# yerfor/Real3DPortrait

Measured on AMD Instinct MI355X. Metric: rendered frames/sec @ 512x512, 48 depth samples, higher is better.
Workload: dtype f32 operands as fp16 hi + lo, fp32 accumulate (SR precision 'f16mx' = the library default, superresolution.DEFAULT_SR_PRECISION; the fp32-class f16x3 is `alt_f16x3`): in block0.conv1, block1.conv0 and block1.conv1 hi*hi runs on the f16 MFMA and the two cross products on the block-scaled 8-bit MFMA

## Files before the change

### real3dportrait_amd/csrc/r3d_render.hip

```cpp

#include <algorithm>
#include "r3d_common.h"
#include "r3d_stamps.h"

namespace r3d {

static constexpr int kC = R3D_FEATURES;
static constexpr int kHid = R3D_HIDDEN;
static constexpr int kOut = R3D_DECODER_OUT;
static constexpr int kWavesPerBlock = 4;

__device__ __forceinline__ void block_absmax_store(float m, float* __restrict__ absmax_part, int block_linear, float* red)
{
#pragma unroll
    for (int d = 32; d >= 1; d >>= 1) m = fmaxf(m, __shfl_xor(m, d));
    const int tid = threadIdx.y * blockDim.x + threadIdx.x, nw = (blockDim.x * blockDim.y) >> 6;
    if ((tid & 63) == 0) red[tid >> 6] = m;
    __syncthreads();
    if (tid == 0) {
        float r = red[0];
        for (int w = 1; w < nw; ++w) r = fmaxf(r, red[w]);
        absmax_part[block_linear] = r;
    }
}
// ... 260 lines not shown
    if ((threadIdx.x & 63) == 0) { red[0][threadIdx.x >> 6] = kmin; red[1][threadIdx.x >> 6] = kmax; red[2][threadIdx.x >> 6] = any ? 1 : 0; }
    __syncthreads();
    if (threadIdx.x == 0) {
        int* p = gstate + kStateHeader + 3 * blockIdx.x;
        p[0] = min(min(red[0][0], red[0][1]), min(red[0][2], red[0][3]));
        p[1] = max(max(red[1][0], red[1][1]), max(red[1][2], red[1][3]));
        p[2] = red[2][0] | red[2][1] | red[2][2] | red[2][3];
    }
}

__device__ __forceinline__ void split8(const float (&x)[8], h8& hi, h8& lo)
{
#pragma unroll
    for (int j = 0; j < 8; ++j) {
        const float v = as_rounded(x[j]);
        const _Float16 a = (_Float16)fminf(fmaxf(v, -65504.f), 65504.f);
        hi[j] = a; lo[j] = (_Float16)(v - (float)a);
    }
}
__device__ __forceinline__ void split8_bounded(const float (&x)[8], h8& hi, h8& lo)
{
#pragma unroll
    for (int j = 0; j < 8; ++j) {
        const float v = as_rounded(x[j]);
        const _Float16 a = (_Float16)v;
        hi[j] = a; lo[j] = (_Float16)(v - (float)a);
    }
}

struct DecoderLds {
    uint4 w1f[4][2][64];
    uint4 w2f[2][2][2][64];
    float w2s[kHid];
    float b1[kHid];
    float b2[kOut];
    float xs3, hs, ys;
};

__device__ __forceinline__ void stage_decoder(DecoderLds& L, const float* __restrict__ w1,
                                              const float* __restrict__ b1, const float* __restrict__ w2,
                                              const float* __restrict__ b2, const DecFold* __restrict__ fold)
{
    const DecFold F = *fold;
    const float kLog2e = 1.4426950408889634f, kLn2 = 0.6931471805599453f;
    const float g1 = 0.17677669529663687f * kLog2e * F.w1s;
    const float g2 = 0.125f;
    const float g2c = g2 * F.w2s;
    for (int i = threadIdx.x; i < 4 * 64; i += blockDim.x) {
        const int l = i & 63, mt = i >> 6;
        float v[8];
#pragma unroll
        for (int j = 0; j < 8; ++j) v[j] = w1[(16 * mt + (l & 15)) * kC + 8 * (l >> 4) + j] * g1;
        h8 hi, lo; split8(v, hi, lo);
        L.w1f[mt][0][l] = *reinterpret_cast<uint4*>(&hi); L.w1f[mt][1][l] = *reinterpret_cast<uint4*>(&lo);
    }
    for (int i = threadIdx.x; i < 2 * 2 * 64; i += blockDim.x) {
        const int l = i & 63, pp = (i >> 6) & 1, ot = i >> 7;
        float v[8];
#pragma unroll
        for (int j = 0; j < 8; ++j)
            v[j] = w2[(1 + 16 * ot + (l & 15)) * kHid + 16 * (2 * pp + (j >> 2)) + 4 * (l >> 4) + (j & 3)] * g2c;
        h8 hi, lo; split8(v, hi, lo);
        L.w2f[ot][pp][0][l] = *reinterpret_cast<uint4*>(&hi); L.w2f[ot][pp][1][l] = *reinterpret_cast<uint4*>(&lo);
    }
    for (int i = threadIdx.x; i < kHid; i += blockDim.x) { L.w2s[i] = w2[i] * (g2 * kLn2); L.b1[i] = b1[i] * kLog2e; }
    for (int i = threadIdx.x; i < kOut; i += blockDim.x) L.b2[i] = i == 0 ? b2[i] : b2[i] * kLog2e * F.b2s;
    if (threadIdx.x == 0) { L.xs3 = F.xs * (1.0f / 3.0f); L.hs = F.hs; L.ys = F.ys; }
}

struct Tap { int idx; float w; };

__device__ __forceinline__ void plane_taps(float u, float v, int H, int W, int plane_base4, Tap t[4])
{
    const float ix = ((u + 1.0f) * (float)W - 1.0f) * 0.5f;
    const float iy = ((v + 1.0f) * (float)H - 1.0f) * 0.5f;
    const float x0f = floorf(ix), y0f = floorf(iy);
    const float fx1 = ix - x0f, fy1 = iy - y0f;
    const float fx0 = (x0f + 1.0f) - ix, fy0 = (y0f + 1.0f) - iy;
    const float xc = fminf(fmaxf(x0f, -2.0f), (float)W + 1.0f);
    const float yc = fminf(fmaxf(y0f, -2.0f), (float)H + 1.0f);
    const int x0 = (int)xc, y0 = (int)yc;
    const bool okc = (xc == x0f) && (yc == y0f);
    const bool vx0 = okc && x0 >= 0 && x0 < W, vx1 = okc && x0 + 1 >= 0 && x0 + 1 < W;
    const bool vy0 = okc && y0 >= 0 && y0 < H, vy1 = okc && y0 + 1 >= 0 && y0 + 1 < H;
    const int xa = min(max(x0, 0), W - 1), xb = min(max(x0 + 1, 0), W - 1);
    const int ya = min(max(y0, 0), H - 1), yb = min(max(y0 + 1, 0), H - 1);
    const int ra = __mul24(ya, W), rb = __mul24(yb, W);
    t[0].idx = plane_base4 + (ra + xa) * 8; t[0].w = (vx0 && vy0) ? fx0 * fy0 : 0.0f;
    t[1].idx = plane_base4 + (ra + xb) * 8; t[1].w = (vx1 && vy0) ? fx1 * fy0 : 0.0f;
    t[2].idx = plane_base4 + (rb + xa) * 8; t[2].w = (vx0 && vy1) ? fx0 * fy1 : 0.0f;
    t[3].idx = plane_base4 + (rb + xb) * 8; t[3].w = (vx1 && vy1) ? fx1 * fy1 : 0.0f;
}

template <int PLANES_IN_FLIGHT, bool TRI = false>
__device__ __forceinline__ void gather_sample(const float4* __restrict__ planes4, int H, int W, int q,
                                              float px, float py, float pz, float scale, float xs3, float x[8], int D = 1)
{
    const float qx = px * scale, qy = py * scale, qz = pz * scale;
    const int HW8 = H * W * 8;
    const float us[3] = {qx, qx, qz}, vs[3] = {qy, qz, qx};
    if constexpr (TRI) {
        const float ws[3] = {qz, qy, qy};
        float accs[3][8];
#pragma unroll
        for (int p = 0; p < 3; ++p)
#pragma unroll
            for (int c = 0; c < 8; ++c) accs[p][c] = 0.0f;
#pragma unroll
        for (int dz = 0; dz < 2; ++dz) {
            Tap t[12];
#pragma unroll
            for (int p = 0; p < 3; ++p) {
                const float iz = ((ws[p] + 1.0f) * (float)D - 1.0f) * 0.5f;
                const float z0f = floorf(iz);
                const float zc = fminf(fmaxf(z0f, -2.0f), (float)D + 1.0f);
                const int z = (int)zc + dz;
                const bool vz = (zc == z0f) && z >= 0 && z < D;
                const float wz = vz ? (dz ? iz - z0f : (z0f + 1.0f) - iz) : 0.0f;
                plane_taps(us[p], vs[p], H, W, (p * D + min(max(z, 0), D - 1)) * HW8 + 2 * q, t + 4 * p);
#pragma unroll
                for (int k = 0; k < 4; ++k) t[4 * p + k].w *= wz;
            }
            float4 lo[12], hi[12];
#pragma unroll
            for (int i = 0; i < 12; ++i) { lo[i] = planes4[t[i].idx]; hi[i] = planes4[t[i].idx + 1]; }
#pragma unroll
            for (int p = 0; p < 3; ++p)
#pragma unroll
                for (int k = 0; k < 4; ++k) {
                    const float w = t[4 * p + k].w;
                    const float4 a = lo[4 * p + k], b = hi[4 * p + k];
                    accs[p][0] += a.x * w; accs[p][1] += a.y * w; accs[p][2] += a.z * w; accs[p][3] += a.w * w;
                    accs[p][4] += b.x * w; accs[p][5] += b.y * w; accs[p][6] += b.z * w; accs[p][7] += b.w * w;
                }
            __builtin_amdgcn_sched_barrier(0);
        }
#pragma unroll
        for (int c = 0; c < 8; ++c) x[c] = (accs[0][c] + accs[1][c] + accs[2][c]) * xs3;
        return;
    }
    float acc[3][8];
    if (PLANES_IN_FLIGHT == 3) {
        Tap t[12];
#pragma unroll
        for (int p = 0; p < 3; ++p) plane_taps(us[p], vs[p], H, W, p * HW8 + 2 * q, t + 4 * p);
        float4 lo[12], hi[12];
#pragma unroll
        for (int i = 0; i < 12; ++i) { lo[i] = planes4[t[i].idx]; hi[i] = planes4[t[i].idx + 1]; }
#pragma unroll
        for (int p = 0; p < 3; ++p) {
#pragma unroll
            for (int c = 0; c < 8; ++c) acc[p][c] = 0.0f;
#pragma unroll
            for (int k = 0; k < 4; ++k) {
                const float w = t[4 * p + k].w;
                const float4 a = lo[4 * p + k], b = hi[4 * p + k];
                acc[p][0] += a.x * w; acc[p][1] += a.y * w; acc[p][2] += a.z * w; acc[p][3] += a.w * w;
                acc[p][4] += b.x * w; acc[p][5] += b.y * w; acc[p][6] += b.z * w; acc[p][7] += b.w * w;
            }
        }
    } else {
        const float4* __restrict__ pl = planes4 + 2 * q;
        const int pq = q < 2 ? q : 2;
        Tap tq[4];
        plane_taps(pq == 2 ? qz : qx, pq == 0 ? qy : (pq == 1 ? qz : qx), H, W, pq * HW8, tq);
#pragma unroll
        for (int p = 0; p < 3; ++p) {
            Tap t[4];
#pragma unroll
            for (int k = 0; k < 4; ++k) {
                t[k].idx = p == 0 ? __builtin_amdgcn_mov_dpp(tq[k].idx, 0x00, 0xF, 0xF, true) : p == 1 ? __builtin_amdgcn_mov_dpp(tq[k].idx, 0x55, 0xF, 0xF, true) : __builtin_amdgcn_mov_dpp(tq[k].idx, 0xAA, 0xF, 0xF, true);
                const int wi = __builtin_bit_cast(int, tq[k].w);
                t[k].w = __builtin_bit_cast(float, p == 0 ? __builtin_amdgcn_mov_dpp(wi, 0x00, 0xF, 0xF, true) : p == 1 ? __builtin_amdgcn_mov_dpp(wi, 0x55, 0xF, 0xF, true) : __builtin_amdgcn_mov_dpp(wi, 0xAA, 0xF, 0xF, true));
            }
            float4 lo[4], hi[4];
#pragma unroll
            for (int i = 0; i < 4; ++i) { lo[i] = pl[t[i].idx]; hi[i] = pl[t[i].idx + 1]; }
#pragma unroll
            for (int c = 0; c < 8; ++c) acc[p][c] = 0.0f;
#pragma unroll
            for (int k = 0; k < 4; ++k) {
                const float w = t[k].w;
                const float4 a = lo[k], b = hi[k];
                acc[p][0] += a.x * w; acc[p][1] += a.y * w; acc[p][2] += a.z * w; acc[p][3] += a.w * w;
                acc[p][4] += b.x * w; acc[p][5] += b.y * w; acc[p][6] += b.z * w; acc[p][7] += b.w * w;
            }
            __builtin_amdgcn_sched_barrier(0);
        }
    }
#pragma unroll
    for (int c = 0; c < 8; ++c) x[c] = (acc[0][c] + acc[1][c] + acc[2][c]) * xs3;
}

struct DecodeState { f32x4 h[4]; };

__device__ __forceinline__ void decode_a(const DecoderLds& L, int lane, const h8 xh, const h8 xl, DecodeState& S, float& sig)
{
    const int q = lane >> 4;
#pragma unroll
    for (int mt = 0; mt < 4; ++mt) {
        f32x4 acc;
        acc[0] = L.b1[16 * mt + 4 * q + 0]; acc[1] = L.b1[16 * mt + 4 * q + 1];
        acc[2] = L.b1[16 * mt + 4 * q + 2]; acc[3] = L.b1[16 * mt + 4 * q + 3];
        uint4 a0 = L.w1f[mt][0][lane], a1 = L.w1f[mt][1][lane];
        const h8 wh = *reinterpret_cast<h8*>(&a0), wl = *reinterpret_cast<h8*>(&a1);
        acc = __builtin_amdgcn_mfma_f32_16x16x32_f16(wl, xh, acc, 0, 0, 0);
        acc = __builtin_amdgcn_mfma_f32_16x16x32_f16(wh, xl, acc, 0, 0, 0);
        acc = __builtin_amdgcn_mfma_f32_16x16x32_f16(wh, xh, acc, 0, 0, 0);
        S.h[mt] = acc;
    }
    float sg = 0.0f;
#pragma unroll
    for (int mt = 0; mt < 4; ++mt)
#pragma unroll
        for (int r = 0; r < 4; ++r) {
            const float x = S.h[mt][r];
            const float sp = __builtin_fmaf(x + fabsf(x), 0.5f, __builtin_amdgcn_logf(1.0f + __builtin_amdgcn_exp2f(-fabsf(x))));
            S.h[mt][r] = sp;
            sg += sp * L.w2s[16 * mt + 4 * q + r];
        }
    sg += __shfl_xor(sg, 16);
    sg += __shfl_xor(sg, 32);
    sig = sg + L.b2[0];
    const float hs = L.hs;
    if (hs != 1.0f) {
#pragma unroll
        for (int mt = 0; mt < 4; ++mt)
#pragma unroll
            for (int r = 0; r < 4; ++r) S.h[mt][r] *= hs;
    }
}

template <int PP>
__device__ __forceinline__ void decode_l2(const DecoderLds& L, int lane, const DecodeState& S, f32x4 (&col)[2])
{
    const int q = lane >> 4;
    if (PP == 0) {
#pragma unroll
        for (int ot = 0; ot < 2; ++ot) {
            col[ot][0] = L.b2[1 + 16 * ot + 4 * q + 0]; col[ot][1] = L.b2[1 + 16 * ot + 4 * q + 1];
            col[ot][2] = L.b2[1 + 16 * ot + 4 * q + 2]; col[ot][3] = L.b2[1 + 16 * ot + 4 * q + 3];
        }
    }
    const float hv[8] = {S.h[2 * PP][0], S.h[2 * PP][1], S.h[2 * PP][2], S.h[2 * PP][3],
                         S.h[2 * PP + 1][0], S.h[2 * PP + 1][1], S.h[2 * PP + 1][2], S.h[2 * PP + 1][3]};
    h8 bh, bl;
    split8_bounded(hv, bh, bl);
#pragma unroll
    for (int ot = 0; ot < 2; ++ot) {
        uint4 a0 = L.w2f[ot][PP][0][lane], a1 = L.w2f[ot][PP][1][lane];
        const h8 wh = *reinterpret_cast<h8*>(&a0), wl = *reinterpret_cast<h8*>(&a1);
        col[ot] = __builtin_amdgcn_mfma_f32_16x16x32_f16(wl, bh, col[ot], 0, 0, 0);
        col[ot] = __builtin_amdgcn_mfma_f32_16x16x32_f16(wh, bl, col[ot], 0, 0, 0);
        col[ot] = __builtin_amdgcn_mfma_f32_16x16x32_f16(wh, bh, col[ot], 0, 0, 0);
    }
    if (PP == 1) {
        const float ys = L.ys;
        if (ys != 1.0f) {
#pragma unroll
            for (int ot = 0; ot < 2; ++ot)
#pragma unroll
                for (int r = 0; r < 4; ++r) col[ot][r] *= ys;
        }
#pragma unroll
        for (int ot = 0; ot < 2; ++ot)
#pragma unroll
            for (int r = 0; r < 4; ++r)
                col[ot][r] = __builtin_amdgcn_rcpf(1.0f + __builtin_amdgcn_exp2f(-col[ot][r])) * 1.002f - 0.001f;
    }
}

__device__ __forceinline__ void decode_tile(const DecoderLds& L, int lane, const h8 xh, const h8 xl, f32x4 (&col)[2], float& sig)
{
    DecodeState S;
    decode_a(L, lane, xh, xl, S, sig);
    decode_l2<0>(L, lane, S, col);
    decode_l2<1>(L, lane, S, col);
}

template <int CTRL, int ROW_MASK = 0xF>
__device__ __forceinline__ float dpp_f(float old, float x) {
    return __builtin_bit_cast(float, __builtin_amdgcn_update_dpp(__builtin_bit_cast(int, old), __builtin_bit_cast(int, x), CTRL, ROW_MASK, 0xF, false));
}
template <int CTRL, int ROW_MASK = 0xF>
__device__ __forceinline__ int dpp_i(int old, int x) { return __builtin_amdgcn_update_dpp(old, x, CTRL, ROW_MASK, 0xF, false); }
__device__ __forceinline__ float wave_incl_mul(float v, int) {
    v *= dpp_f<0x111>(1.0f, v); v *= dpp_f<0x112>(1.0f, v); v *= dpp_f<0x114>(1.0f, v); v *= dpp_f<0x118>(1.0f, v);
    v *= dpp_f<0x142, 0xA>(1.0f, v); v *= dpp_f<0x143, 0xC>(1.0f, v);
    return v;
}
__device__ __forceinline__ float wave_incl_add(float v, int) {
    v += dpp_f<0x111>(0.0f, v); v += dpp_f<0x112>(0.0f, v); v += dpp_f<0x114>(0.0f, v); v += dpp_f<0x118>(0.0f, v);
    v += dpp_f<0x142, 0xA>(0.0f, v); v += dpp_f<0x143, 0xC>(0.0f, v);
    return v;
}
__device__ __forceinline__ int wave_incl_add_i(int v) {
    v += dpp_i<0x111>(0, v); v += dpp_i<0x112>(0, v); v += dpp_i<0x114>(0, v); v += dpp_i<0x118>(0, v);
    v += dpp_i<0x142, 0xA>(0, v); v += dpp_i<0x143, 0xC>(0, v);
    return v;
}
__device__ __forceinline__ float wave_shift_up1(float v, float first) { return dpp_f<0x138>(first, v); }
__device__ __forceinline__ float lane63(float v) { return __builtin_bit_cast(float, __builtin_amdgcn_readlane(__builtin_bit_cast(int, v), 63)); }
__device__ __forceinline__ float wave_sum(float v) { return lane63(wave_incl_add(v, 0)); }
__device__ __forceinline__ void wave_lds_sync() {
    __builtin_amdgcn_fence(__ATOMIC_ACQ_REL, "wavefront");
    __builtin_amdgcn_wave_barrier();
}

struct XchLds { uint4 v[2][64]; };
__device__ __forceinline__ int gather_q(int lane) { return lane & 3; }
__device__ __forceinline__ int gather_s(int lane) { return lane >> 2; }
__device__ __forceinline__ void gather_to_mfma(XchLds& E, int lane, const float (&X)[8], h8& xh, h8& xl)
{
    split8_bounded(X, xh, xl);
    const int gs = lane >> 2, gq = lane & 3, q = lane >> 4, s = lane & 15;
    const int wi = 16 * gq + (gs ^ (2 * gq)), ri = 16 * q + (s ^ (2 * q));
    E.v[0][wi] = *reinterpret_cast<uint4*>(&xh);
    E.v[1][wi] = *reinterpret_cast<uint4*>(&xl);
    wave_lds_sync();
    uint4 rh = E.v[0][ri], rl = E.v[1][ri];
    wave_lds_sync();
    xh = *reinterpret_cast<h8*>(&rh);
    xl = *reinterpret_cast<h8*>(&rl);
}

template <int NS, int NCD>
struct RayLds {
    float t[NS];
    float sg[NS];
    float ts[NS];
    float ss[NS];
    float wv[NS];
    float om[NS];
    float cdf[NCD];
    int cnt[NS];
};

struct FeatLds { uint4 v[2][2 * 64]; };

typedef __amdgpu_buffer_rsrc_t PlaneRsrc;
template <int NB = 2>
struct TileGather {
    f32x4 lo[NB][4], hi[NB][4];
    float tw[NB][4];
    Tap tq[4];
    float acc[8];
    __device__ __forceinline__ void start(int H, int W, int q, float px, float py, float pz, float scale)
    {
        const float qx = px * scale, qy = py * scale, qz = pz * scale;
        const int pq = q < 2 ? q : 2;
        plane_taps(pq == 2 ? qz : qx, pq == 0 ? qy : (pq == 1 ? qz : qx), H, W, pq * H * W * 8, tq);
#pragma unroll
        for (int k = 0; k < 4; ++k) tq[k].idx *= 16;
    }
    template <int P, int B>
    __device__ __forceinline__ void issue(const PlaneRsrc rsrc, unsigned qoff)
    {
#pragma unroll
        for (int k = 0; k < 4; ++k) {
            const int wbits = __builtin_bit_cast(int, tq[k].w);
            const unsigned off = (unsigned)(P == 0 ? __builtin_amdgcn_mov_dpp(tq[k].idx, 0x00, 0xF, 0xF, true) : P == 1 ? __builtin_amdgcn_mov_dpp(tq[k].idx, 0x55, 0xF, 0xF, true) : __builtin_amdgcn_mov_dpp(tq[k].idx, 0xAA, 0xF, 0xF, true)) + qoff;
            tw[B][k] = __builtin_bit_cast(float, P == 0 ? __builtin_amdgcn_mov_dpp(wbits, 0x00, 0xF, 0xF, true) : P == 1 ? __builtin_amdgcn_mov_dpp(wbits, 0x55, 0xF, 0xF, true) : __builtin_amdgcn_mov_dpp(wbits, 0xAA, 0xF, 0xF, true));
            lo[B][k] = __builtin_bit_cast(f32x4, __builtin_amdgcn_raw_buffer_load_b128(rsrc, (int)off, 0, 0));
            hi[B][k] = __builtin_bit_cast(f32x4, __builtin_amdgcn_raw_buffer_load_b128(rsrc, (int)(off + 16u), 0, 0));
        }
    }
    template <int B>
    __device__ __forceinline__ void pin(f32x4& d0, f32x4& d1)
    {
        asm volatile("" : "+v"(lo[B][0]), "+v"(lo[B][1]), "+v"(lo[B][2]), "+v"(lo[B][3]), "+v"(hi[B][0]), "+v"(hi[B][1]), "+v"(hi[B][2]), "+v"(hi[B][3]),
                          "+v"(d0), "+v"(d1));
    }
    template <int P, int B>
    __device__ __forceinline__ void consume()
    {
        float pa[8];
#pragma unroll
        for (int c = 0; c < 8; ++c) pa[c] = 0.0f;
#pragma unroll
        for (int k = 0; k < 4; ++k) {
            const float w = tw[B][k];
            const f32x4 a4 = lo[B][k], b4 = hi[B][k];
            pa[0] += a4[0] * w; pa[1] += a4[1] * w; pa[2] += a4[2] * w; pa[3] += a4[3] * w;
            pa[4] += b4[0] * w; pa[5] += b4[1] * w; pa[6] += b4[2] * w; pa[7] += b4[3] * w;
        }
#pragma unroll
        for (int c = 0; c < 8; ++c) acc[c] = P == 0 ? pa[c] : acc[c] + pa[c];
    }
    __device__ __forceinline__ void finish(FeatLds& F, int slot, int wi, float xs3)
    {
        float X[8];
#pragma unroll
        for (int c = 0; c < 8; ++c) X[c] = acc[c] * xs3;
        h8 xh, xl;
        split8_bounded(X, xh, xl);
        F.v[0][slot * 64 + wi] = *reinterpret_cast<uint4*>(&xh);
        F.v[1][slot * 64 + wi] = *reinterpret_cast<uint4*>(&xl);
    }
};

template <int NT, int GPF, bool TRI, int NB = 2, typename DepthFn, typename FirstFn>
__device__ __forceinline__ void decode_pass(FeatLds& F, const DecoderLds& dec, const float4* __restrict__ P, int H, int W, int D, int lane,
                                            float ox, float oy, float oz, float dx, float dy, float dz, float scale, float xs3,
                                            DepthFn depth_of, FirstFn first_done, f32x4 (&col0)[NT], f32x4 (&col1)[NT], float (&sig)[NT], f32x4* gp = nullptr)
{
    const int gq = lane & 3, gs = lane >> 2, q = lane >> 4, s = lane & 15;
    const int wi = 16 * gq + (gs ^ (2 * gq)), ri = 16 * q + (s ^ (2 * q));
    const uint64_t pb = (uint64_t)(uintptr_t)P;
    void* pu = reinterpret_cast<void*>((uintptr_t)(((uint64_t)(unsigned)__builtin_amdgcn_readfirstlane((int)(pb >> 32)) << 32) |
                                                   (unsigned)__builtin_amdgcn_readfirstlane((int)(pb & 0xffffffffu))));
    const PlaneRsrc pl = __builtin_amdgcn_make_buffer_rsrc(pu, 0, __builtin_amdgcn_readfirstlane(3 * (TRI ? D : 1) * H * W * 128), 0x00020000);
    const unsigned qoff = 32u * (unsigned)gq;
    TileGather<NB> g;
    auto gather_whole = [&](int t) {
        const float tg = depth_of(t);
        if constexpr (TRI) {
            float X[8]; h8 xh, xl;
            gather_sample<GPF, true>(P, H, W, gq, ox + tg * dx, oy + tg * dy, oz + tg * dz, scale, xs3, X, D);
            split8_bounded(X, xh, xl);
            F.v[0][(t & 1) * 64 + wi] = *reinterpret_cast<uint4*>(&xh); F.v[1][(t & 1) * 64 + wi] = *reinterpret_cast<uint4*>(&xl);
        } else {
            f32x4 z0 = {0.f, 0.f, 0.f, 0.f}, z1 = z0;
            g.start(H, W, gq, ox + tg * dx, oy + tg * dy, oz + tg * dz, scale);
            g.template issue<0, 0>(pl, qoff);
            if constexpr (NB == 2) {
                g.template issue<1, 1>(pl, qoff);
                g.template pin<0>(z0, z1); g.template consume<0, 0>();
                g.template issue<2, 0>(pl, qoff);
                g.template pin<1>(z0, z1); g.template consume<1, 1>();
                g.template pin<0>(z0, z1); g.template consume<2, 0>();
            } else {
                g.template pin<0>(z0, z1); g.template consume<0, 0>();
                g.template issue<1, 0>(pl, qoff);
                g.template pin<0>(z0, z1); g.template consume<1, 0>();
                g.template issue<2, 0>(pl, qoff);
                g.template pin<0>(z0, z1); g.template consume<2, 0>();
            }
            g.finish(F, t & 1, wi, xs3);
        }
    };
    gather_whole(0);
    first_done();
#pragma unroll
    for (int t = 0; t < NT; ++t) {
        wave_lds_sync();
        uint4 rh = F.v[0][(t & 1) * 64 + ri], rl4 = F.v[1][(t & 1) * 64 + ri];
        const h8 xh = *reinterpret_cast<h8*>(&rh), xl = *reinterpret_cast<h8*>(&rl4);
        const bool more = t + 1 < NT;
        DecodeState S;
        f32x4 c2[2];
        if (more && !TRI) {
            const float tg = depth_of(t + 1);
            g.start(H, W, gq, ox + tg * dx, oy + tg * dy, oz + tg * dz, scale);
            g.template issue<0, 0>(pl, qoff);
        }
        __builtin_amdgcn_sched_barrier(0);
        decode_a(dec, lane, xh, xl, S, sig[t]);
        __builtin_amdgcn_sched_barrier(0);
        if (more && !TRI) { g.template pin<0>(S.h[0], S.h[3]); g.template consume<0, 0>(); g.template issue<1, 0>(pl, qoff); }
        __builtin_amdgcn_sched_barrier(0);
        decode_l2<0>(dec, lane, S, c2);
        __builtin_amdgcn_sched_barrier(0);
        if (more && !TRI) { g.template pin<0>(c2[0], c2[1]); g.template consume<1, 0>(); g.template issue<2, 0>(pl, qoff); }
        __builtin_amdgcn_sched_barrier(0);
        decode_l2<1>(dec, lane, S, c2);
        __builtin_amdgcn_sched_barrier(0);
        if (more && !TRI) { g.template pin<0>(c2[0], c2[1]); g.template consume<2, 0>(); g.finish(F, (t + 1) & 1, wi, xs3); }
        if (more && TRI) gather_whole(t + 1);
        if (gp) { gp[(2 * t) * 64] = c2[0]; gp[(2 * t + 1) * 64] = c2[1]; }
        else { col0[t] = c2[0]; col1[t] = c2[1]; }
        __builtin_amdgcn_sched_barrier(0);
    }
}

template <int SLOTS>
__device__ __forceinline__ void march(const float* T, const float* S, float* wv, int n, int lane,
                                      float& wsum, float& dsum)
{
    float carry = 1.0f, ws = 0.0f, ds = 0.0f;
#pragma unroll
    for (int sl = 0; sl < SLOTS; ++sl) {
        const int i = sl * 64 + lane;
        const bool act = i < n - 1;
        const int i0 = act ? i : 0;
        const float t0 = T[i0], t1 = T[i0 + 1], s0 = S[i0], s1 = S[i0 + 1];
        const float delta = t1 - t0;
        const float dmid = (s0 + s1) * 0.5f;
        const float tmid = (t0 + t1) * 0.5f;
        const float sp = softplus20(dmid - 1.0f);
        const float alpha = one_minus_exp_neg(sp * delta);
        const float om1 = act ? (1.0f - alpha + 1e-10f) : 1.0f;
        const float incl = wave_incl_mul(om1, lane);
        const float excl = wave_shift_up1(incl, 1.0f);
        const float w = act ? alpha * (carry * excl) : 0.0f;
        carry *= lane63(incl);
        if (act) wv[i] = w;
        ws += w;
        ds += w * tmid;
    }
    wsum = wave_sum(ws);
    dsum = wave_sum(ds);
}

constexpr bool render_shape_parks(int ntc, int ntf) { return ntf > 0 && ntc > 3; }
constexpr int render_park_tiles(int ntc, int ntf) { return render_shape_parks(ntc, ntf) ? 2 * (ntc + ntf) : 0; }

struct RenderArgs {
    const float4* planes4; int N, H, W, M, D;
    const float* w1; const float* b1; const float* w2; const float* b2;
    const float* origins; const float* dirs;
    const float* cam_c2w; const float* cam_K; int cam_R;
    uint2* split_out; const float* split_scale; size_t split_scale_stride;
    const float* ray_start; const float* ray_end; const uint8_t* valid;
    int* gstate; int nlimit_blocks;
    int Nc, Nf; float scale; int white_back;
    const float* noise_c; const float* u_f; unsigned long long seed;
    const DecFold* fold;
    float* rgb; float* depth; float* wsum; int rgb_cm;
    unsigned long long* clk;
    f32x4* park_g;
};

struct RayIter {
    int strips, n, c, row, sa, sb, sc, R, strip, N, M, col0;
    long long lin, lstride, nrays;
    __device__ __forceinline__ void init(const RenderArgs& a, int R_, int wave)
    {
        const int wv = __builtin_amdgcn_readfirstlane(wave);
        R = R_; N = a.N; M = a.M;
        strips = (R > 0 && (R & 7) == 0 && (gridDim.x & 7) == 0) ? 1 : 0;
        if (strips) {
            const unsigned xcd = blockIdx.x & 7, bx = blockIdx.x >> 3, nbx = gridDim.x >> 3;
            strip = R >> 3; col0 = (int)xcd * strip;
            const unsigned per_img = (unsigned)strip * (unsigned)R;
            const unsigned w0 = bx * kWavesPerBlock + (unsigned)wv, st = nbx * kWavesPerBlock;
            n = (int)(w0 / per_img); const unsigned rem = w0 - (unsigned)n * per_img;
            c = (int)(rem / (unsigned)R); row = (int)(rem - (unsigned)c * (unsigned)R);
            sa = (int)(st / per_img); const unsigned srem = st - (unsigned)sa * per_img;
            sb = (int)(srem / (unsigned)R); sc = (int)(srem - (unsigned)sb * (unsigned)R);
        } else {
            nrays = (long long)a.N * a.M;
            lin = (long long)blockIdx.x * kWavesPerBlock + wv;
            lstride = (long long)gridDim.x * kWavesPerBlock;
        }
    }
    __device__ __forceinline__ bool get(int& ray, int& img) const
    {
        if (strips) { if (n >= N) return false; img = n; ray = n * M + row * R + col0 + c; return true; }
        if (lin >= nrays) return false;
        ray = (int)lin; img = ray / M; return true;
    }
    __device__ __forceinline__ void advance()
    {
        if (strips) {
            row += sc; if (row >= R) { row -= R; ++c; }
            c += sb;   if (c >= strip) { c -= strip; ++n; }
            n += sa;
        } else lin += lstride;
    }
};

template <int NTC, int NTF, int OCC, int GPF, bool TRI = false>
__global__ __launch_bounds__(256, OCC) void render_kernel(RenderArgs a, int R)
{
    constexpr int SLOTS = (16 * (NTC + NTF) + 63) / 64;
    constexpr int CSLOTS = (16 * NTC + 63) / 64;
    constexpr int FSLOTS = NTF > 0 ? (16 * NTF + 63) / 64 : 1;
    typedef RayLds<16 * (NTC + NTF) + 8, 16 * NTC + 8> RayL;
    __shared__ __attribute__((aligned(16))) DecoderLds dec;
    __shared__ __attribute__((aligned(16))) RayL rl[kWavesPerBlock];
    __shared__ __attribute__((aligned(16))) FeatLds feat[kWavesPerBlock];
    constexpr bool PARK = NTF > 0 && NTC <= 3;
    constexpr bool GPARK = render_shape_parks(NTC, NTF);
    __shared__ __attribute__((aligned(16))) f32x4 park[PARK ? kWavesPerBlock : 1][PARK ? 2 * NTC : 1][64];

    stage_decoder(dec, a.w1, a.b1, a.w2, a.b2, a.fold);
    __syncthreads();
    const float xs3 = dec.xs3;

    const int lane = threadIdx.x & 63, wave = threadIdx.x >> 6;
    const int q = lane >> 4, s = lane & 15;
    const int gs = gather_s(lane);
    RayL& L = rl[wave];
    FeatLds& F = feat[wave];
    int pmin = 0x7fffffff, pmax = (int)0x80000000, pany = 0;
    for (int b = lane; b < a.nlimit_blocks; b += 64) {
        const int* p = a.gstate + kStateHeader + 3 * b;
        pmin = min(pmin, p[0]); pmax = max(pmax, p[1]); pany |= p[2];
    }
#pragma unroll
    for (int d = 32; d >= 1; d >>= 1) { pmin = min(pmin, __shfl_xor(pmin, d)); pmax = max(pmax, __shfl_xor(pmax, d)); pany |= __shfl_xor(pany, d); }
    const float gmin_start = ord2f(pmin), gmax_start = ord2f(pmax);
    const bool any_valid = pany != 0;
    const int Nc_all = a.Nc;
    float run_min = INFINITY, run_max = -INFINITY;
    R3D_STAMP_DECL;
    int st_rays_ = 0; (void)st_rays_;
    if (blockIdx.x == (gridDim.x >> 1) && threadIdx.x == 0) clk_begin(kernarg_clk<RenderArgs>());

    RayIter it;
    it.init(a, R, wave);
    for (;; it.advance()) {
        typedef const __attribute__((address_space(4))) RenderArgs* KArgs;
        KArgs ap = (KArgs)__builtin_amdgcn_kernarg_segment_ptr();
        asm volatile("" : "+s"(ap));
        const auto& A = *ap;
        const int Nc = NTF > 0 ? A.Nc : Nc_all, Nf = A.Nf, S = Nc + Nf;
        int ray, n;
        if (!it.get(ray, n)) break;
        ++st_rays_;
        R3D_STAMP(7);
        const float4* P = A.planes4 + (size_t)n * 3 * (TRI ? A.D : 1) * A.H * A.W * 8;
        float ox, oy, oz, dx, dy, dz;
        if (A.cam_c2w) {
            float o3[3], d3[3];
            make_ray(A.cam_c2w + 16 * n, A.cam_K + 9 * n, A.cam_R, ray - n * A.M, o3, d3);
            ox = o3[0]; oy = o3[1]; oz = o3[2]; dx = d3[0]; dy = d3[1]; dz = d3[2];
        } else {
            ox = A.origins[3 * (size_t)ray]; oy = A.origins[3 * (size_t)ray + 1]; oz = A.origins[3 * (size_t)ray + 2];
            dx = A.dirs[3 * (size_t)ray]; dy = A.dirs[3 * (size_t)ray + 1]; dz = A.dirs[3 * (size_t)ray + 2];
        }
        float start = A.ray_start[ray], end = A.ray_end[ray];
        if (!A.valid[ray] && any_valid) { start = gmin_start; end = gmax_start; }

        const float span = end - start;
        const float delta = span / (float)(Nc - 1);
        float tc[NTC];
#pragma unroll
        for (int nt = 0; nt < NTC; ++nt) {
            const int k = 16 * nt + s;
            const bool act = k < Nc;
            const float step = (float)k / (float)(Nc - 1);
            float u = 0.0f;
            if (act) u = A.noise_c ? A.noise_c[(size_t)ray * Nc + k] : hash_uniform(A.seed, 0, (uint64_t)ray * Nc + k);
            tc[nt] = act ? (start + step * span) + u * delta : start;
        }
        R3D_STAMP(0);
        f32x4 colc[2][NTC];
        float sigc[NTC];
        f32x4* gpark = nullptr;
        if constexpr (GPARK) gpark = A.park_g + ((size_t)(blockIdx.x * kWavesPerBlock + wave) * render_park_tiles(NTC, NTF)) * 64 + lane;
        {
            if (q == 0) {
#pragma unroll
                for (int nt = 0; nt < NTC; ++nt) {
                    const int k = 16 * nt + s;
                    if (k < Nc) L.t[k] = tc[nt];
                }
            }
            wave_lds_sync();
            auto dof = [&](int t) { const int k = 16 * t + gs; return k < Nc ? L.t[k] : start; };
            decode_pass<NTC, GPF, TRI, (OCC >= 3 ? 1 : 2)>(F, dec, P, A.H, A.W, A.D, lane, ox, oy, oz, dx, dy, dz, A.scale, xs3, dof,
                                                           [&]() { R3D_STAMP(8); }, colc[0], colc[1], sigc, gpark);
        }
        constexpr bool parked = PARK;
        if (parked) {
#pragma unroll
            for (int nt = 0; nt < NTC; ++nt) { park[PARK ? wave : 0][PARK ? 2 * nt : 0][lane] = colc[0][nt]; park[PARK ? wave : 0][PARK ? 2 * nt + 1 : 0][lane] = colc[1][nt]; }
        }

        if (q == 0) {
#pragma unroll
            for (int nt = 0; nt < NTC; ++nt) {
                const int k = 16 * nt + s;
                if (k < Nc) L.sg[k] = sigc[nt];
            }
        }
        wave_lds_sync();
        R3D_STAMP(1);

        float wsum, dsum;
        f32x4 colf[2][NTF > 0 ? NTF : 1];
        bool fine_done = false;
        if constexpr (NTF > 0) { if (Nf > 0) {
            fine_done = true;
            march<CSLOTS>(L.t, L.sg, L.wv, Nc, lane, wsum, dsum);
            wave_lds_sync();
            const int ns = Nc - 3;
            float omega[CSLOTS], tot = 0.0f;
#pragma unroll
            for (int sl = 0; sl < CSLOTS; ++sl) {
                const int i = sl * 64 + lane;
                const bool act = i < ns;
                const int i0 = act ? i : 0;
                const float w0 = L.wv[i0], w1v = L.wv[i0 + 1], w2v = L.wv[i0 + 2];
                const float sv = (fmaxf(w0, w1v) + fmaxf(w1v, w2v)) * 0.5f + 0.01f;
                omega[sl] = act ? sv + 1e-5f : 0.0f;
                tot += omega[sl];
            }
            tot = wave_sum(tot);
            float carry = 0.0f;
            if (lane == 0) L.cdf[0] = 0.0f;
#pragma unroll
            for (int sl = 0; sl < CSLOTS; ++sl) {
                const int i = sl * 64 + lane;
                const float incl = wave_incl_add(omega[sl] / tot, lane);
                if (i < ns) L.cdf[i + 1] = carry + incl;
                carry += lane63(incl);
            }
            wave_lds_sync();
#pragma unroll
            for (int sl = 0; sl < FSLOTS; ++sl) {
                const int j = sl * 64 + lane;
                if (j < Nf) {
                    const float u = A.u_f ? A.u_f[(size_t)ray * Nf + j] : hash_uniform(A.seed, 1, (uint64_t)ray * Nf + j);
                    int lo = 0, hi = ns + 1;
                    while (lo < hi) { const int mid = (lo + hi) >> 1; if (L.cdf[mid] <= u) lo = mid + 1; else hi = mid; }
                    const int below = max(lo - 1, 0), above = min(lo, ns);
                    const float cb = L.cdf[below], ca = L.cdf[above];
                    const float bb = 0.5f * (L.t[below] + L.t[below + 1]);
                    const float ba = 0.5f * (L.t[above] + L.t[above + 1]);
                    float den = ca - cb;
                    if (den < 1e-5f) den = 1.0f;
                    L.t[Nc + j] = bb + (u - cb) / den * (ba - bb);
                }
            }
            wave_lds_sync();
            R3D_STAMP(2);
            float sigf[NTF > 0 ? NTF : 1];
            {
                auto dof = [&](int t) { const int k = 16 * t + gs; return L.t[Nc + (k < Nf ? k : 0)]; };
                decode_pass<(NTF > 0 ? NTF : 1), GPF, TRI, (OCC >= 3 ? 1 : 2)>(F, dec, P, A.H, A.W, A.D, lane, ox, oy, oz, dx, dy, dz, A.scale, xs3, dof,
                                                                             [&]() { R3D_STAMP(9); }, colf[0], colf[1], sigf, GPARK ? gpark + 2 * NTC * 64 : nullptr);
            }
            if (q == 0) {
#pragma unroll
                for (int nt = 0; nt < NTF; ++nt) {
                    const int k = 16 * nt + s;
                    if (k < Nf) L.sg[Nc + k] = sigf[nt];
                }
            }
            wave_lds_sync();
            R3D_STAMP(3);
            int rank[SLOTS];
            bool fast = true;
#pragma unroll
            for (int sl = 0; sl < CSLOTS; ++sl) {
                const int i = sl * 64 + lane;
                const bool act = i < Nc - 1;
                fast = fast && (!act || L.t[act ? i : 0] <= L.t[act ? i + 1 : 0]);
            }
            fast = __all(fast);
            if (fast) {
#pragma unroll
                for (int sl = 0; sl < CSLOTS + 1; ++sl) { const int i = sl * 64 + lane; if (i <= Nc) L.cnt[i] = 0; }
                wave_lds_sync();
                int rf[FSLOTS];
#pragma unroll
                for (int sl = 0; sl < FSLOTS; ++sl) {
                    const int j = sl * 64 + lane;
                    const bool act = j < Nf;
                    const float tj = L.t[Nc + (act ? j : 0)];
                    int lo = 0, hi = Nc;
                    while (lo < hi) { const int mid = (lo + hi) >> 1; if (L.t[mid] <= tj) lo = mid + 1; else hi = mid; }
                    int f = 0;
                    for (int k = 0; k < Nf; ++k) f += (L.t[Nc + k] < tj) ? 1 : 0;
                    rf[sl] = lo + f;
                    if (act) atomicAdd(&L.cnt[lo], 1);
                }
                wave_lds_sync();
                int carry = 0;
                int rc[CSLOTS];
#pragma unroll
                for (int sl = 0; sl < CSLOTS; ++sl) {
                    const int i = sl * 64 + lane;
                    int v = i < Nc ? L.cnt[i] : 0;
                    v = wave_incl_add_i(v);
                    rc[sl] = i + carry + v;
                    carry += __builtin_amdgcn_readlane(v, 63);
                }
                wave_lds_sync();
#pragma unroll
                for (int sl = 0; sl < CSLOTS; ++sl) { const int i = sl * 64 + lane; if (i < Nc) L.cnt[rc[sl]] = i; }
#pragma unroll
                for (int sl = 0; sl < FSLOTS; ++sl) { const int j = sl * 64 + lane; if (j < Nf) L.cnt[rf[sl]] = Nc + j; }
                wave_lds_sync();
                bool ok = true;
#pragma unroll
                for (int sl = 0; sl < CSLOTS; ++sl) { const int i = sl * 64 + lane; if (i < Nc) ok = ok && L.cnt[rc[sl]] == i; }
#pragma unroll
                for (int sl = 0; sl < FSLOTS; ++sl) { const int j = sl * 64 + lane; if (j < Nf) ok = ok && L.cnt[rf[sl]] == Nc + j; }
                fast = __all(ok);
                if (fast) {
#pragma unroll
                    for (int sl = 0; sl < CSLOTS; ++sl) { const int i = sl * 64 + lane; if (i < Nc) L.cnt[i] = rc[sl]; }
#pragma unroll
                    for (int sl = 0; sl < FSLOTS; ++sl) { const int j = sl * 64 + lane; if (j < Nf) L.cnt[Nc + j] = rf[sl]; }
                    wave_lds_sync();
#pragma unroll
                    for (int sl = 0; sl < SLOTS; ++sl) {
                        const int i = sl * 64 + lane;
                        rank[sl] = L.cnt[i < S ? i : 0];
                    }
                }
            }
            if (!fast) {
                if (lane == 0) atomicAdd(&g_merge_fallbacks, 1u);
#pragma unroll
                for (int sl = 0; sl < SLOTS; ++sl) {
                    const int i = sl * 64 + lane;
                    const float ti = L.t[i < S ? i : 0];
                    int cnt = 0;
                    for (int j = 0; j < S; ++j) {
                        const float tj = L.t[j];
                        cnt += (tj < ti || (tj == ti && j < i)) ? 1 : 0;
                    }
                    rank[sl] = cnt;
                }
            }
#pragma unroll
            for (int sl = 0; sl < SLOTS; ++sl) {
                const int i = sl * 64 + lane;
                if (i < S) { L.ts[rank[sl]] = L.t[i]; L.ss[rank[sl]] = L.sg[i]; }
            }
            wave_lds_sync();
            R3D_STAMP(4);
            march<SLOTS>(L.ts, L.ss, L.wv, S, lane, wsum, dsum);
            wave_lds_sync();
#pragma unroll
            for (int sl = 0; sl < SLOTS; ++sl) {
                const int i = sl * 64 + lane, r = rank[sl];
                if (i < S) {
                    const float wl = r > 0 ? L.wv[r - 1] : 0.0f;
                    const float wr = r < S - 1 ? L.wv[r] : 0.0f;
                    L.om[i] = 0.5f * (wl + wr);
                }
            }
        } }
        if (!fine_done) {
            march<CSLOTS>(L.t, L.sg, L.wv, Nc, lane, wsum, dsum);
            wave_lds_sync();
#pragma unroll
            for (int sl = 0; sl < CSLOTS; ++sl) {
                const int i = sl * 64 + lane;
                if (i < Nc) {
                    const float wl = i > 0 ? L.wv[i - 1] : 0.0f;
                    const float wr = i < Nc - 1 ? L.wv[i] : 0.0f;
                    L.om[i] = 0.5f * (wl + wr);
                }
            }
        }
        wave_lds_sync();
        R3D_STAMP(5);

        f32x4 acc[2];
        acc[0] = (f32x4){0.f, 0.f, 0.f, 0.f};
        acc[1] = acc[0];
#pragma unroll
        for (int nt = 0; nt < NTC; ++nt) {
            const int k = 16 * nt + s;
            const float om = k < Nc ? L.om[k] : 0.0f;
            f32x4 cc0 = colc[0][nt], cc1 = colc[1][nt];
            if (parked) { cc0 = park[PARK ? wave : 0][PARK ? 2 * nt : 0][lane]; cc1 = park[PARK ? wave : 0][PARK ? 2 * nt + 1 : 0][lane]; }
            if constexpr (GPARK) { cc0 = gpark[(2 * nt) * 64]; cc1 = gpark[(2 * nt + 1) * 64]; }
            acc[0] += cc0 * om;
            acc[1] += cc1 * om;
        }
        if constexpr (NTF > 0) {
#pragma unroll
            for (int nt = 0; nt < NTF; ++nt) {
                const int k = 16 * nt + s;
                const float om = (fine_done && k < Nf) ? L.om[Nc + k] : 0.0f;
                f32x4 cf0 = colf[0][nt], cf1 = colf[1][nt];
                if constexpr (GPARK) { cf0 = gpark[(2 * (NTC + nt)) * 64]; cf1 = gpark[(2 * (NTC + nt) + 1) * 64]; }
                acc[0] += cf0 * om;
                acc[1] += cf1 * om;
            }
        }
#pragma unroll
        for (int ot = 0; ot < 2; ++ot)
#pragma unroll
            for (int r = 0; r < 4; ++r) {
                float v = acc[ot][r];
                v += dpp_f<0x128>(0.0f, v); v += dpp_f<0x124>(0.0f, v); v += dpp_f<0x122>(0.0f, v); v += dpp_f<0x121>(0.0f, v);
                if (A.white_back) v = v + 1.0f - wsum;
                acc[ot][r] = v * 2.0f - 1.0f;
            }
        if (s == 0 && A.split_out) {
            const float* sc = A.split_scale + (size_t)n * A.split_scale_stride;
            const size_t pix = (size_t)(ray - n * A.M), plane = (size_t)(kC / 8) * A.M;
#pragma unroll
            for (int ot = 0; ot < 2; ++ot) {
                const float4 s4 = *reinterpret_cast<const float4*>(sc + 16 * ot + 4 * q);
                const float sv[4] = {s4.x, s4.y, s4.z, s4.w};
                typedef _Float16 h4v __attribute__((ext_vector_type(4)));
                h4v hi, lo;
#pragma unroll
                for (int r = 0; r < 4; ++r) {
                    _Float16 hh, ll;
                    split_scaled(acc[ot][r], sv[r], hh, ll);
                    hi[r] = hh; lo[r] = ll;
                }
                uint2* dst = A.split_out + (((size_t)n * 2 * plane + (size_t)(2 * ot + (q >> 1)) * A.M + pix) * 2 + (q & 1));
                dst[0] = *reinterpret_cast<uint2*>(&hi);
                dst[2 * plane] = *reinterpret_cast<uint2*>(&lo);
            }
        }
        if (s == 0) {
            if (A.rgb_cm) {
                float* o = A.rgb + ((size_t)n * kC + 4 * q) * A.M + (ray - n * A.M);
#pragma unroll
                for (int r = 0; r < 4; ++r) { o[(size_t)r * A.M] = acc[0][r]; o[(size_t)(16 + r) * A.M] = acc[1][r]; }
            } else {
                float4* o4 = reinterpret_cast<float4*>(A.rgb + (size_t)ray * kC);
                o4[q] = make_float4(acc[0][0], acc[0][1], acc[0][2], acc[0][3]);
                o4[4 + q] = make_float4(acc[1][0], acc[1][1], acc[1][2], acc[1][3]);
            }
        }
        float lmin = INFINITY, lmax = -INFINITY;
#pragma unroll
        for (int sl = 0; sl < SLOTS; ++sl) {
            const int i = sl * 64 + lane;
            if (i < S) { const float v = L.t[i]; lmin = fminf(lmin, v); lmax = fmaxf(lmax, v); }
        }
        run_min = fminf(run_min, lmin); run_max = fmaxf(run_max, lmax);
        if (lane == 0) {
            if (A.depth) A.depth[ray] = dsum / wsum;
            A.wsum[ray] = wsum;
        }
        wave_lds_sync();
        R3D_STAMP(6);
    }
    R3D_STAMP_FLUSH(10, st_rays_);
    if (blockIdx.x == (gridDim.x >> 1) && threadIdx.x == 0) clk_end(kernarg_clk<RenderArgs>());
#pragma unroll
    for (int d = 32; d >= 1; d >>= 1) {
        run_min = fminf(run_min, __shfl_xor(run_min, d));
        run_max = fmaxf(run_max, __shfl_xor(run_max, d));
    }
    if (lane == 0 && run_min <= run_max) {
        atomicMin(&a.gstate[3], f2ord(run_min));
        atomicMax(&a.gstate[4], f2ord(run_max));
    }
}

template <bool TRI>
__global__ __launch_bounds__(256, 2) void run_model_kernel(const float4* __restrict__ planes4, int N, int H, int W, int D,
                                                          const float* w1, const float* b1, const float* w2, const float* b2,
                                                          const float* __restrict__ coords, int npts, float scale,
                                                          float* __restrict__ rgb, float* __restrict__ sigma, const DecFold* __restrict__ fold)
{
    __shared__ __attribute__((aligned(16))) DecoderLds dec;
    __shared__ __attribute__((aligned(16))) XchLds xch[kWavesPerBlock];
    stage_decoder(dec, w1, b1, w2, b2, fold);
    __syncthreads();
    const float xs3 = dec.xs3;
    const int lane = threadIdx.x & 63, wave = threadIdx.x >> 6;
    const int q = lane >> 4, s = lane & 15;
    const int gq = gather_q(lane), gs = gather_s(lane);
    XchLds& E = xch[wave];
    const long long total = (long long)N * npts;
    const long long chunks = (total + 63) / 64;
    for (long long ch = (long long)blockIdx.x * kWavesPerBlock + wave; ch < chunks; ch += (long long)gridDim.x * kWavesPerBlock) {
        long long idx[4];
        f32x4 col[2][4];
        float sig[4];
#pragma unroll
        for (int nt = 0; nt < 4; ++nt) {
            idx[nt] = ch * 64 + 16 * nt + s;
            const long long ig = ch * 64 + 16 * nt + gs;
            const long long ii = ig < total ? ig : total - 1;
            const int n = (int)(ii / npts);
            const float4* P = planes4 + (size_t)n * 3 * (TRI ? D : 1) * H * W * 8;
            float X[8];
            f32x4 c2[2];
            h8 xh, xl;
            gather_sample<3, TRI>(P, H, W, gq, coords[3 * ii], coords[3 * ii + 1], coords[3 * ii + 2], scale, xs3, X, D);
            gather_to_mfma(E, lane, X, xh, xl);
            decode_tile(dec, lane, xh, xl, c2, sig[nt]);
            col[0][nt] = c2[0]; col[1][nt] = c2[1];
            __builtin_amdgcn_sched_barrier(0);
        }
#pragma unroll
        for (int nt = 0; nt < 4; ++nt) {
            if (idx[nt] < total) {
                float4* o4 = reinterpret_cast<float4*>(rgb + (size_t)idx[nt] * kC);
                o4[q] = make_float4(col[0][nt][0], col[0][nt][1], col[0][nt][2], col[0][nt][3]);
                o4[4 + q] = make_float4(col[1][nt][0], col[1][nt][1], col[1][nt][2], col[1][nt][3]);
                if (q == 0) sigma[idx[nt]] = sig[nt];
            }
        }
    }
}

static constexpr int kMaxGrid = 512;
static inline size_t align64(size_t v) { return (v + 63) & ~(size_t)63; }

#define R3D_RENDER_PLANE_SHAPES(X) X(1, 0) X(1, 1) X(2, 0) X(2, 1) X(2, 2) X(3, 0) X(3, 1) X(3, 2) X(3, 3) X(4, 0) X(6, 0) X(4, 4) X(6, 6)
#define R3D_RENDER_TRI_SHAPES(X) X(6, 0) X(3, 3) X(6, 6)

struct RenderShape {
    int ntc, ntf; bool tri;
    void (*kernel)(RenderArgs, int);
    bool parks() const { return render_shape_parks(ntc, ntf); }
};
static const RenderShape kRenderShapes[] = {
#define R3D_SHAPE(C_, F_) {C_, F_, false, render_kernel<C_, F_, 2, 1>},
    R3D_RENDER_PLANE_SHAPES(R3D_SHAPE)
#undef R3D_SHAPE
#define R3D_SHAPE(C_, F_) {C_, F_, true, render_kernel<C_, F_, 2, 3, true>},
    R3D_RENDER_TRI_SHAPES(R3D_SHAPE)
#undef R3D_SHAPE
};
#define R3D_SHAPE(C_, F_) render_park_tiles(C_, F_),
static constexpr int kRenderParkTilesMax = std::max({R3D_RENDER_PLANE_SHAPES(R3D_SHAPE) R3D_RENDER_TRI_SHAPES(R3D_SHAPE)});
#undef R3D_SHAPE
static_assert(kRenderParkTilesMax == 24, "r3d_render_workspace_bytes: the parking room per wave is 24 tiles of 64 f32x4");

static const RenderShape* find_render_shape(bool tri, int ntc, int ntf)
{
    for (const RenderShape& s : kRenderShapes)
        if (s.tri == tri && s.ntc == ntc && s.ntf == ntf) return &s;
    return nullptr;
}

static const RenderShape& pick_render_shape(int Nc, int Nf, int triplane_depth)
{
    const int ntc = (Nc + 15) / 16, ntf = (Nf + 15) / 16;
    const bool tri = triplane_depth > 1;
    if (const RenderShape* s = find_render_shape(tri, ntc, ntf)) return *s;
    static const int cover[3][2] = {{6, 0}, {3, 3}, {4, 4}};
    for (const int* c : cover)
        if (ntc <= c[0] && ntf <= c[1] && (ntf == 0) == (c[1] == 0))
            if (const RenderShape* s = find_render_shape(tri, c[0], c[1])) return *s;
    return *find_render_shape(tri, 6, 6);
}

static int render_grid(size_t nrays)
{
    const size_t max_blocks = ((nrays + kWavesPerBlock - 1) / kWavesPerBlock + 7) / 8 * 8;
    return max_blocks < (size_t)kMaxGrid ? (int)max_blocks : kMaxGrid;
}
static size_t render_park_bytes(size_t nrays, int Nc, int Nf)
{
    const bool parks = pick_render_shape(Nc, Nf, 1).parks() || pick_render_shape(Nc, Nf, 2).parks();
    return parks ? (size_t)render_grid(nrays) * kWavesPerBlock * kRenderParkTilesMax * 64 * sizeof(f32x4) : 0;
}

static_assert(sizeof(DecFold) <= 64, "the fold record's slot is 64 bytes");
struct RenderWorkspaceLayout { size_t gstate, ray_start, ray_end, fold, partials, park, total; };
static RenderWorkspaceLayout render_workspace_layout(bool rays, size_t nrays, size_t park_bytes)
{
    RenderWorkspaceLayout L;
    size_t o = 0;
    L.gstate = o; if (rays) o += align64((kStateHeader + 3 * ((nrays + kLimitsBlock - 1) / kLimitsBlock)) * sizeof(int));
    L.ray_start = o; if (rays) o += nrays * sizeof(float);
    L.ray_end = o; if (rays) o += nrays * sizeof(float);
    const size_t rays_end = o;
    L.fold = o = align64(o); o += 64;
    L.partials = o; o += kAbsmaxBlocks * sizeof(float);
    L.park = o; o += park_bytes;
    L.total = rays_end + (rays ? 64 : 0) + (o - L.fold);
    return L;
}

struct PlaneBound { const float* partials; int count; };
static PlaneBound plane_bound(const float* plane_absmax, int n_plane_absmax, const float* planes_nhwc, size_t plane_floats, float* own, hipStream_t st)
{
    if (plane_absmax && n_plane_absmax > 0) return {plane_absmax, n_plane_absmax};
    hipLaunchKernelGGL(plane_absmax_kernel, dim3(kAbsmaxBlocks), dim3(256), 0, st, reinterpret_cast<const float4*>(planes_nhwc), plane_floats / 4, own);
    return {own, kAbsmaxBlocks};
}

static constexpr long long kIntMax = 2147483647;
static constexpr size_t kTapByteLimit = (size_t)1 << 32, kGatherLimit = (size_t)1 << 31;
static bool planes_fit(int H, int W, int depth, size_t texel_units, size_t limit)
{
    return H < (1 << 24) && W < (1 << 24) && (size_t)H * W * 3 * depth * texel_units < limit;
}

static int check_planes_decoder(const char* what, const float* planes_nhwc, int N, int H, int W, int triplane_depth,
                                const float* w1, const float* b1, const float* w2, const float* b2, float box_warp)
{
    if (!planes_nhwc || !w1 || !b1 || !w2 || !b2) { set_error("%s: NULL pointer (planes_nhwc, w1, b1, w2, b2)", what); return R3D_ERR_INVALID_ARG; }
    if (N <= 0 || H <= 1 || W <= 1 || triplane_depth < 1 || triplane_depth > 16 || !(box_warp > 0.f)) {
        set_error("%s: bad shape (N > 0, H, W > 1, 1 <= triplane_depth <= 16, box_warp > 0)", what); return R3D_ERR_INVALID_ARG;
    }
    return R3D_OK;
}

}

using namespace r3d;

R3D_STAMP_READER(r3d_debug_stamps)

static inline bool nhwc32_fast_path(const void* a, const void* b, const void* c, int C, int HW, int depth, int add_flip)
{
    const bool aligned16 = !(((uintptr_t)a | (uintptr_t)b | (uintptr_t)c) & 15);
    return C == 32 && depth == 1 && add_flip == 0 && (HW & 63) == 0 && aligned16;
}
extern "C" size_t r3d_planes_absmax_partials(int N, int C, int H, int W, int depth)
{
    if (N <= 0 || C <= 0 || H <= 0 || W <= 0 || depth < 1) return 0;
    const size_t HW = (size_t)H * W;
    return ((HW + 31) / 32) * ((C + 31) / 32) * (size_t)N * 3 * depth;
// ... 153 lines not shown
```

Measured before the change: 1701.

## Pre-sort fine-sample uniforms with a wave bitonic sort to simplify merge ranking

Sorts the importance-sampling uniforms in registers with a DPP/swizzle bitonic network before the coarse pass. Inverse-CDF sampling is monotone, so the fine depths come out already ordered. That lets the merge use rank j+lo directly, which removes the O(Nf) per-lane count loop and the scatter/verify round-trip through LDS. A strict-ordering check on the fine depths keeps the O(S^2) fallback for ties or non-monotone cases. The sort adds shuffle work per ray and depends on the positive-float-as-int ordering of the uniforms.

```diff
diff --git a/real3dportrait_amd/csrc/r3d_render.hip b/real3dportrait_amd/csrc/r3d_render.hip
--- a/real3dportrait_amd/csrc/r3d_render.hip
+++ b/real3dportrait_amd/csrc/r3d_render.hip
@@ -586,6 +586,49 @@
 __device__ __forceinline__ float wave_shift_up1(float v, float first) { return dpp_f<0x138>(first, v); }
 __device__ __forceinline__ float lane63(float v) { return __builtin_bit_cast(float, __builtin_amdgcn_readlane(__builtin_bit_cast(int, v), 63)); }
 __device__ __forceinline__ float wave_sum(float v) { return lane63(wave_incl_add(v, 0)); }
+template <int M>
+__device__ __forceinline__ int lane_xor(int v, int lane)
+{
+    if constexpr (M == 1) return __builtin_amdgcn_mov_dpp(v, 0xB1, 0xF, 0xF, true);
+    else if constexpr (M == 2) return __builtin_amdgcn_mov_dpp(v, 0x4E, 0xF, 0xF, true);
+    else if constexpr (M == 3) return __builtin_amdgcn_mov_dpp(v, 0x1B, 0xF, 0xF, true);
+    else if constexpr (M == 7) return __builtin_amdgcn_mov_dpp(v, 0x141, 0xF, 0xF, true);
+    else if constexpr (M == 8) return __builtin_amdgcn_mov_dpp(v, 0x128, 0xF, 0xF, true);
+    else if constexpr (M == 15) return __builtin_amdgcn_mov_dpp(v, 0x140, 0xF, 0xF, true);
+    else if constexpr (M == 4 || M == 16 || M == 31) return __builtin_amdgcn_ds_swizzle(v, (M << 10) | 0x1F);
+    else { static_assert(M == 32 || M == 63, "no exchange for this lane mask"); return __builtin_amdgcn_ds_bpermute((lane ^ M) << 2, v); }
+}
+template <int M, int BIT, int FS>
+__device__ __forceinline__ void sort_step(int (&v)[FS], int lane)
+{
+#pragma unroll
+    for (int sl = 0; sl < FS; ++sl) {
+        const int p = lane_xor<M>(v[sl], lane);
+        v[sl] = (lane & BIT) ? max(v[sl], p) : min(v[sl], p);
+    }
+}
+template <int J, int FS>
+__device__ __forceinline__ void sort_tail(int (&v)[FS], int lane)
+{
+    if constexpr (J >= 1) { sort_step<J, J>(v, lane); sort_tail<J / 2>(v, lane); }
+}
+template <int K, int FS>
+__device__ __forceinline__ void sort_stages(int (&v)[FS], int lane)
+{
+    if constexpr (K >= 2) { sort_stages<K / 2>(v, lane); sort_step<K - 1, K / 2>(v, lane); sort_tail<K / 4>(v, lane); }
+}
+template <int FS>
+__device__ __forceinline__ void wave_sort(int (&v)[FS], int lane)
+{
+    static_assert(FS == 1 || FS == 2, "one or two keys per lane");
+    sort_stages<64>(v, lane);
+    if constexpr (FS == 2) {
+        const int p0 = lane_xor<63>(v[1], lane), p1 = lane_xor<63>(v[0], lane);
+        v[0] = min(v[0], p0); v[1] = max(v[1], p1);
+        sort_tail<32>(v, lane);
+    }
+}
+
 __device__ __forceinline__ void wave_lds_sync() {
     __builtin_amdgcn_fence(__ATOMIC_ACQ_REL, "wavefront");
     __builtin_amdgcn_wave_barrier();
@@ -934,6 +977,21 @@
             }
             wave_lds_sync();
             auto dof = [&](int t) { const int k = 16 * t + gs; return k < Nc ? L.t[k] : start; };
+            if constexpr (NTF > 0) {
+                int key[FSLOTS];
+#pragma unroll
+                for (int sl = 0; sl < FSLOTS; ++sl) {
+                    const int j = sl * 64 + lane;
+                    key[sl] = 0x7fffffff;
+                    if (j < Nf) key[sl] = __float_as_int(A.u_f ? A.u_f[(size_t)ray * Nf + j] : hash_uniform(A.seed, 1, (uint64_t)ray * Nf + j));
+                }
+                int sl_lane = lane;
+                asm volatile("" : "+v"(sl_lane));
+                wave_sort(key, sl_lane);
+#pragma unroll
+                for (int sl = 0; sl < FSLOTS; ++sl) { const int j = sl * 64 + lane; if (j < Nf) L.t[Nc + j] = __int_as_float(key[sl]); }
+                wave_lds_sync();
+            }
             decode_pass<NTC, GPF, TRI, (OCC >= 3 ? 1 : 2)>(F, dec, P, A.H, A.W, A.D, lane, ox, oy, oz, dx, dy, dz, A.scale, xs3, dof,
                                                            [&]() { R3D_STAMP(8); }, colc[0], colc[1], sigc, gpark);
         }
@@ -987,7 +1045,7 @@
             for (int sl = 0; sl < FSLOTS; ++sl) {
                 const int j = sl * 64 + lane;
                 if (j < Nf) {
-                    const float u = A.u_f ? A.u_f[(size_t)ray * Nf + j] : hash_uniform(A.seed, 1, (uint64_t)ray * Nf + j);
+                    const float u = L.t[Nc + j];
                     int lo = 0, hi = ns + 1;
                     while (lo < hi) { const int mid = (lo + hi) >> 1; if (L.cdf[mid] <= u) lo = mid + 1; else hi = mid; }
                     const int below = max(lo - 1, 0), above = min(lo, ns);
@@ -1024,6 +1082,12 @@
                 const bool act = i < Nc - 1;
                 fast = fast && (!act || L.t[act ? i : 0] <= L.t[act ? i + 1 : 0]);
             }
+#pragma unroll
+            for (int sl = 0; sl < FSLOTS; ++sl) {
+                const int j = sl * 64 + lane;
+                const bool act = j < Nf - 1;
+                fast = fast && (!act || L.t[Nc + (act ? j : 0)] < L.t[Nc + (act ? j + 1 : 0)]);
+            }
             fast = __all(fast);
             if (fast) {
 #pragma unroll
@@ -1037,9 +1101,7 @@
                     const float tj = L.t[Nc + (act ? j : 0)];
                     int lo = 0, hi = Nc;
                     while (lo < hi) { const int mid = (lo + hi) >> 1; if (L.t[mid] <= tj) lo = mid + 1; else hi = mid; }
-                    int f = 0;
-                    for (int k = 0; k < Nf; ++k) f += (L.t[Nc + k] < tj) ? 1 : 0;
-                    rf[sl] = lo + f;
+                    rf[sl] = j + lo;
                     if (act) atomicAdd(&L.cnt[lo], 1);
                 }
                 wave_lds_sync();
@@ -1055,27 +1117,14 @@
                 }
                 wave_lds_sync();
 #pragma unroll
-                for (int sl = 0; sl < CSLOTS; ++sl) { const int i = sl * 64 + lane; if (i < Nc) L.cnt[rc[sl]] = i; }
-#pragma unroll
-                for (int sl = 0; sl < FSLOTS; ++sl) { const int j = sl * 64 + lane; if (j < Nf) L.cnt[rf[sl]] = Nc + j; }
+                for (int sl = 0; sl < CSLOTS; ++sl) { const int i = sl * 64 + lane; if (i < Nc) L.cnt[i] = rc[sl]; }
+#pragma unroll
+                for (int sl = 0; sl < FSLOTS; ++sl) { const int j = sl * 64 + lane; if (j < Nf) L.cnt[Nc + j] = rf[sl]; }
                 wave_lds_sync();
-                bool ok = true;
-#pragma unroll
-                for (int sl = 0; sl < CSLOTS; ++sl) { const int i = sl * 64 + lane; if (i < Nc) ok = ok && L.cnt[rc[sl]] == i; }
-#pragma unroll
-                for (int sl = 0; sl < FSLOTS; ++sl) { const int j = sl * 64 + lane; if (j < Nf) ok = ok && L.cnt[rf[sl]] == Nc + j; }
-                fast = __all(ok);
-                if (fast) {
-#pragma unroll
-                    for (int sl = 0; sl < CSLOTS; ++sl) { const int i = sl * 64 + lane; if (i < Nc) L.cnt[i] = rc[sl]; }
-#pragma unroll
-                    for (int sl = 0; sl < FSLOTS; ++sl) { const int j = sl * 64 + lane; if (j < Nf) L.cnt[Nc + j] = rf[sl]; }
-                    wave_lds_sync();
-#pragma unroll
-                    for (int sl = 0; sl < SLOTS; ++sl) {
-                        const int i = sl * 64 + lane;
-                        rank[sl] = L.cnt[i < S ? i : 0];
-                    }
+#pragma unroll
+                for (int sl = 0; sl < SLOTS; ++sl) {
+                    const int i = sl * 64 + lane;
+                    rank[sl] = L.cnt[i < S ? i : 0];
                 }
             }
             if (!fast) {
```

After: 1708 (median of 6 runs). Within noise of the previous version (+0.4%).
